# StractOrg/stract

Measured on NVIDIA H100. Metric: webgraph_edges_per_sec_per_centrality_iter, higher is better.
Workload: dtype u8

## Files before the change

### stract_b200/csrc/api_graph.cu

```cuda
#include "graph.cuh"

#include <algorithm>
#include <vector>

namespace sb200 {
static thread_local char t_err[1024] = "";
std::atomic<uint64_t> g_launches{0};
thread_local cudaStream_t t_pool_stream = nullptr;
void set_error(const char* fmt, ...) {
  va_list ap; va_start(ap, fmt);
  vsnprintf(t_err, sizeof(t_err), fmt, ap);
  va_end(ap);
}
int hb_alloc_state(sb200_graph* g);
int hb_reset(sb200_graph* g);
int hb_step(sb200_graph* g, sb200_iter_stats* st);
int hb_step_launch(sb200_graph* g, bool with_barrier);
int hb_step_finish(sb200_graph* g, sb200_iter_stats* st);
int hb_barrier(sb200_graph* g);
__global__ void k_owned_flags(const uint32_t* __restrict__ inv, const uint32_t* __restrict__ sub, uint64_t N, uint32_t world, uint32_t rank,
                              uint8_t* owned, uint32_t* sub_out) {
  const uint64_t r = blockIdx.x * (uint64_t)blockDim.x + threadIdx.x;
  if (r >= N) return;
  const uint32_t v = inv[r];
  if (owned) owned[r] = (world <= 1 || ((v >> 5) % world) == rank) ? 1 : 0;
  if (sub_out) sub_out[r] = sub ? sub[v] : (world <= 1 ? 1u : 0xFFFFFFFFu >> (32 - world));
}
int hb_result(sb200_graph* g, uint64_t* id_lo, uint64_t* id_hi, double* cent, uint64_t cap, uint64_t* len);
int hb_registers(sb200_graph* g, uint64_t first, uint64_t count, uint8_t* out);
int hb_ranked(sb200_graph* g, int ties_desc, uint64_t* id_lo, uint64_t* id_hi, double* cent, uint64_t cap, uint64_t* len);
int hb_kahan(sb200_graph* g, uint64_t first, uint64_t count, double* sum, double* err);
}
using namespace sb200;

uint64_t sb200_graph::hbm_bytes() const {
  return id_lo.bytes() + id_hi.bytes() + perm.bytes() + inv.bytes() + row_ptr.bytes() + col.bytes() + fwd_ptr.bytes() +
         fwd_dst.bytes() + item_row.bytes() + item_start.bytes() + partial.bytes() + regs[0].bytes() + regs[1].bytes() +
         bm[0].bytes() + bm[1].bytes() + size_cache.bytes() + kahan_sum.bytes() + kahan_err.bytes() +
         frontier_list.bytes() + frontier_off.bytes() + frontier_scan.bytes() + cub_tmp.bytes() + counters.bytes() + sub_mask.bytes() + sync_page.bytes();
}

extern "C" {

const char* sb200_last_error(void) { return t_err; }
#ifndef SB200_EMU
const char* sb200_version(void) { return "stract_b200 0.1 (sm_90a)"; }
#else
const char* sb200_version(void) { return "stract_b200 0.1 CPU SIMT emulation (tests/emu, tests only)"; }
#endif
uint64_t sb200_kernel_launch_count(void) { return g_launches.load(); }

#define SB_ENTER(g)                                            \
  if (!(g)) SB_FAIL(SB200_EINVAL, "NULL graph handle");        \
  SB_CUDA(cudaSetDevice((g)->device))

int sb200_graph_create(const uint64_t* from_lo, const uint64_t* from_hi, const uint64_t* to_lo, const uint64_t* to_hi,
                       const uint64_t* rel_flags, uint64_t n_edges, uint64_t skipped_rel_mask, int device, int rank,
                       int world_size, sb200_graph** out) {
  if (!out) SB_FAIL(SB200_EINVAL, "out is NULL");
  *out = nullptr;
  if (world_size < 1 || world_size > 64 || rank < 0 || rank >= world_size)
// ... 106 lines not shown
  SB_CUDA(cudaEventRecord(g->ev_run1, g->stream));
  SB_CUDA(cudaStreamSynchronize(g->stream));
  cudaEventElapsedTime(&g->last_run_ms, g->ev_run0, g->ev_run1);
  if (iters_done) *iters_done = g->t;
  return SB200_OK;
}

int sb200_hyperball_last_run_ms(sb200_graph* g, float* ms) {
  if (!g || !ms) SB_FAIL(SB200_EINVAL, "NULL argument");
  *ms = g->last_run_ms;
  return SB200_OK;
}

int sb200_hyperball_set_profiling(sb200_graph* g, int on) {
  if (!g) SB_FAIL(SB200_EINVAL, "NULL graph handle");
  g->profiling = on != 0;
  for (int f = 0; f < sb200_graph::F_COUNT; f++) { g->prof_launches[f] = 0; g->prof_ms[f] = 0; g->prof_bytes[f] = 0; g->prof_used[f] = false; }
  return SB200_OK;
}

int sb200_hyperball_get_profile(sb200_graph* g, sb200_kernel_prof* out, uint32_t cap, uint32_t* n) {
  if (!g || !n) SB_FAIL(SB200_EINVAL, "NULL argument");
  static const char* names[sb200_graph::F_COUNT] = {"k_pull_warp<dense>", "k_pull_quad<dense>", "k_pull_warp<frontier>",
                                                     "k_pull_quad<frontier>", "k_pull_merge", "k_push", "k_finalize"};
  uint32_t k = 0;
  for (int f = 0; f < sb200_graph::F_COUNT; f++) {
    if (out && k < cap) {
      memset(&out[k], 0, sizeof(out[k]));
      strncpy(out[k].name, names[f], sizeof(out[k].name) - 1);
      out[k].launches = g->prof_launches[f]; out[k].ms = g->prof_ms[f]; out[k].alg_bytes = g->prof_bytes[f];
    }
    k++;
  }
  *n = k;
  return SB200_OK;
}

int sb200_hyperball_result(sb200_graph* g, uint64_t* id_lo, uint64_t* id_hi, double* centrality, uint64_t cap, uint64_t* len) {
  SB_ENTER(g);
  if (!len) SB_FAIL(SB200_EINVAL, "len is NULL");
  if (centrality && (!id_lo || !id_hi)) SB_FAIL(SB200_EINVAL, "id outputs are NULL");
  return hb_result(g, id_lo, id_hi, centrality, cap, len);
}

int sb200_hyperball_ranked(sb200_graph* g, int ties_desc, uint64_t* id_lo, uint64_t* id_hi, double* centrality, uint64_t cap, uint64_t* len) {
  SB_ENTER(g);
  if (!len) SB_FAIL(SB200_EINVAL, "len is NULL");
// ... 229 lines not shown
```

### stract_b200/csrc/graph.cuh

```cuda
#pragma once
#include "common.cuh"

namespace sb200 {
constexpr int MAX_PEERS = 15;
struct PeerOut { uint4* newr[MAX_PEERS]; uint32_t* bmc[MAX_PEERS]; const uint32_t* sub; int n; uint32_t world, rank; uint8_t prank[MAX_PEERS + 1]; };
constexpr int SYNC_SLOTS = 128;
struct SyncView { unsigned long long* local; unsigned long long* peer[MAX_PEERS]; int n; uint32_t world, rank; };
}

struct sb200_graph {
  int device = 0, rank = 0, world = 1;
  cudaStream_t stream = nullptr;
  cudaEvent_t ev0 = nullptr, ev1 = nullptr;
  uint64_t N = 0, E_in = 0, E_kept = 0, E_local = 0;
  uint64_t row_begin = 0, row_end = 0;
  uint64_t n_pos = 0;
  bool has_fwd = false;
  int reuse = 0;
  double stage_ms = 0;

  sb200::DevBuf<uint64_t> id_lo, id_hi;
  sb200::DevBuf<uint32_t> perm, inv;
  sb200::DevBuf<uint32_t> self_bm;
  sb200::DevBuf<uint32_t> row_ptr, col;
  uint32_t col_base = 0;
  sb200::DevBuf<uint32_t> fwd_ptr, fwd_dst;
  sb200::DevBuf<uint32_t> row_ranges_host_dummy;
  uint64_t range_begins[65] = {0};

  uint64_t warp_row_begin = 0, warp_row_end = 0;
  uint64_t quad_row_begin = 0, quad_row_end = 0;
  uint64_t n_items = 0;
  uint64_t n_multi_rows = 0;
  sb200::DevBuf<uint32_t> owned_items;
  uint64_t n_owned_items = 0;
  sb200::DevBuf<uint32_t> item_row, item_start;
  sb200::DevBuf<uint4> partial;
  uint64_t n_multi_items = 0;

  sb200::DevBuf<uint8_t> regs[2];
  sb200::DevBuf<uint32_t> bm[2];
  sb200::DevBuf<uint64_t> size_cache;
  sb200::DevBuf<double> kahan_sum, kahan_err;
  sb200::DevBuf<uint32_t> frontier_list, frontier_off;
  sb200::DevBuf<unsigned long long> frontier_scan;
  sb200::DevBuf<uint8_t> cub_tmp;
  sb200::DevBuf<unsigned long long> counters;
  unsigned long long* h_counters = nullptr;
  int cur = 0;
  int bcur = 0;
  uint32_t t = 0;
  bool has_changes = true;
  uint64_t n_changed_prev = 0, frontier_edges_prev = 0;
  bool exchange_pending = false;
  int n_peers = 0;
  bool p2p = false;
  bool peers_ipc = true;
  void* peer_regs[2][sb200::MAX_PEERS] = {{nullptr}};
  void* peer_bm[2][sb200::MAX_PEERS] = {{nullptr}};
  int peer_rank[sb200::MAX_PEERS] = {0};
  bool publish_all = false;
  sb200::DevBuf<uint32_t> sub_mask;
  uint64_t n_subscribed = 0;
  sb200::DevBuf<unsigned long long> sync_page;
  void* peer_sync[sb200::MAX_PEERS] = {nullptr};
  uint64_t sync_epoch = 0;
  bool step_in_flight = false, step_with_barrier = false;
  int step_mode = 0;
  double dense_frac = 0.35, push_div = 48.0;
  int force_mode = -1;
  uint64_t l2_window_bytes = 0;

  enum { F_PULL_WARP_DENSE, F_PULL_QUAD_DENSE, F_PULL_WARP_FRONT, F_PULL_QUAD_FRONT, F_PULL_MERGE, F_PUSH, F_FINALIZE, F_COUNT };
  bool profiling = false;
  uint64_t prof_launches[F_COUNT] = {0};
  double prof_ms[F_COUNT] = {0}, prof_bytes[F_COUNT] = {0};
  cudaEvent_t prof_ev[F_COUNT][2] = {{nullptr}};
  int sm_count = 0;
  int opt_side_ctas = -1, opt_owned_list = -1;
  cudaStream_t side_stream = nullptr;
  cudaEvent_t ev_fork = nullptr, ev_join = nullptr, side_prof[2] = {nullptr, nullptr};
  bool side_prof_used = false;
  int side_prof_family = 0;
  bool prof_used[F_COUNT] = {false};
  double prof_step_bytes[F_COUNT] = {0};
  uint64_t E_warp = 0, E_quad = 0;
  double own_frac = 1.0;
  cudaEvent_t ev_run0 = nullptr, ev_run1 = nullptr;
  float last_run_ms = 0;

  uint64_t hbm_bytes() const;
};

namespace sb200 {
constexpr int QUAD_MAX_DEG = 32;
constexpr int CHUNK_EDGES = 1024;
// ... 6 lines not shown
```

### stract_b200/csrc/hyperball.cu

```cuda
#include <chrono>
#include "graph.cuh"
#include "../../include/sb200_hll_tables.h"

#ifndef SB200_EMU
#include <cub/cub.cuh>
#endif
#include <algorithm>
#include <cmath>
#include <cstdlib>

namespace sb200 {

struct HllTables {
  double raw[SB200_HLL_P5_LEN];
  double bias[SB200_HLL_P5_LEN];
  double lc[65];
};
__constant__ HllTables c_tab;
static bool g_tab_loaded[64] = {false};

int load_tables(int device) {
  if (device >= 0 && device < 64 && g_tab_loaded[device]) return SB200_OK;
  static HllTables h;
  for (int i = 0; i < SB200_HLL_P5_LEN; i++) { h.raw[i] = SB200_HLL_RAW_P5[i]; h.bias[i] = SB200_HLL_BIAS_P5[i]; }
// ... 45 lines not shown
        idx = right ? ir : il;
      } else if (il >= 0) { right = false; idx = il; }
      else { right = true; idx = ir; }
      bsum = __dadd_rn(bsum, tab->bias[idx]);
      if (right) ir = (idx < LEN - 1) ? idx + 1 : -1;
      else il = (idx > 0) ? idx - 1 : -1;
    }
    e_star = __dsub_rn(e, __ddiv_rn(bsum, 6.0));
  }
  const double h = (zeros != 0) ? tab->lc[zeros] : e_star;
  const double pick = (h <= 40.0) ? h : e_star;
  if (!(pick == pick) || pick <= 0.0) return 0ull;
  if (pick >= 18446744073709551616.0) return 0xFFFFFFFFFFFFFFFFull;
  return (uint64_t)__double2ull_rz(pick);
}

__device__ __forceinline__ void kahan_add(double& sum, double& err, double rhs) {
  const double y = __dsub_rn(rhs, err);
  const double t = __dadd_rn(sum, y);
  err = __dsub_rn(__dsub_rn(t, sum), y);
  sum = t;
}

__global__ void k_hb_init(const uint64_t* __restrict__ id_lo, const uint32_t* __restrict__ perm, uint64_t N,
                          uint4* r0, uint4* r1, uint64_t* size_cache, double* ksum, double* kerr) {
  __shared__ HllTables tab;
  for (int i = threadIdx.x; i < (int)(sizeof(HllTables) / 8); i += blockDim.x) ((double*)&tab)[i] = ((const double*)&c_tab)[i];
  __syncthreads();
  uint64_t v = blockIdx.x * (uint64_t)blockDim.x + threadIdx.x;
  if (v >= N) return;
  const uint64_t hash = id_lo[perm[v]] * 11400714819323198549ull;
  const uint32_t j = (uint32_t)(hash >> 58);
  const uint64_t wv = hash << 6;
  const uint32_t p = (wv == 0 ? 64u : (uint32_t)__clzll((long long)wv)) + 1u;
  uint32_t w[16];
#pragma unroll
  for (int i = 0; i < 16; i++) w[i] = 0;
#pragma unroll
  for (int i = 0; i < 16; i++) if ((int)(j >> 2) == i) w[i] = p << (8 * (j & 3));
#pragma unroll
  for (int q = 0; q < 4; q++) {
    uint4 x = make_uint4(w[4 * q], w[4 * q + 1], w[4 * q + 2], w[4 * q + 3]);
    r0[v * 4 + q] = x; r1[v * 4 + q] = x;
  }
  size_cache[v] = hll64_size(w, &tab);
  ksum[v] = 0.0; kerr[v] = 0.0;
}
__global__ void k_bm_fill(uint32_t* bm, uint64_t N, uint64_t words) {
  uint64_t i = blockIdx.x * (uint64_t)blockDim.x + threadIdx.x;
  if (i >= words) return;
  uint64_t first = i * 32;
  uint32_t m = 0xFFFFFFFFu;
  if (first + 32 > N) m = (N > first) ? ((1u << (N - first)) - 1u) : 0u;
  bm[i] = m;
}

__device__ __forceinline__ bool owned_row(const PeerOut& o, uint32_t row) {
  return o.world <= 1u || ((row >> 5) % o.world) == o.rank;
}
__device__ __forceinline__ void publish_row(uint4* __restrict__ newr, uint32_t* __restrict__ bm_cur, const PeerOut& peers,
                                            uint32_t row, uint32_t sub, uint4 acc, bool write, bool changed) {
  if (write) newr[(uint64_t)row * 4 + sub] = acc;
  if (changed && sub == 0) atomicOr(bm_cur + (row >> 5), 1u << (row & 31));
  if (!write || peers.n == 0) return;
  const uint32_t want = peers.sub ? __ldg(peers.sub + row) : 0xFFFFFFFFu;
  for (int p = 0; p < peers.n; p++) {
    if ((want >> peers.prank[p]) & 1u) peers.newr[p][(uint64_t)row * 4 + sub] = acc;
  }
}

__device__ __forceinline__ bool bm_test(const uint32_t* __restrict__ bm, uint32_t v) {
  return (__ldg(bm + (v >> 5)) >> (v & 31)) & 1u;
}

template <bool FRONTIER>
__device__ __forceinline__ void quad_rows(uint64_t row, bool live, uint32_t sub, uint32_t lane,
    const uint32_t* __restrict__ row_ptr, const uint32_t* __restrict__ col, uint32_t col_base,
    const uint4* __restrict__ oldr, uint4* __restrict__ newr,
    const uint32_t* __restrict__ bm_prev, uint32_t* __restrict__ bm_cur, const PeerOut& peers) {
  const uint32_t e0 = live ? row_ptr[row] - col_base : 0u, e1 = live ? row_ptr[row + 1] - col_base : 0u;
  const uint4 own = oldr[row * 4 + sub];
  uint4 acc = own;
  const unsigned qmask = 0xFu << (lane & ~3u);
  const uint32_t self = (uint32_t)row;
  uint32_t nxt = (e0 + sub < e1) ? ld_stream_u32(col + e0 + sub) : self;
  for (uint32_t e = e0; e < e1; e += 4) {
    uint32_t mine = nxt;
    nxt = (e + 4 + sub < e1) ? ld_stream_u32(col + e + 4 + sub) : self;
    if (FRONTIER) mine = bm_test(bm_prev, mine) ? mine : self;
    const uint32_t i0 = __shfl_sync(qmask, mine, 0, 4);
    const uint32_t i1 = __shfl_sync(qmask, mine, 1, 4);
    const uint32_t i2 = __shfl_sync(qmask, mine, 2, 4);
    const uint32_t i3 = __shfl_sync(qmask, mine, 3, 4);
    const uint4 v0 = oldr[(uint64_t)i0 * 4 + sub];
    const uint4 v1 = oldr[(uint64_t)i1 * 4 + sub];
    const uint4 v2 = oldr[(uint64_t)i2 * 4 + sub];
    const uint4 v3 = oldr[(uint64_t)i3 * 4 + sub];
    acc = vmax_u8x16(vmax_u8x16(acc, v0), vmax_u8x16(vmax_u8x16(v1, v2), v3));
  }
  const unsigned ball = __ballot_sync(0xffffffffu, ne_u4(acc, own));
  const bool changed = ((ball >> (lane & ~3u)) & 0xFu) != 0u;
  if (!live) return;
  publish_row(newr, bm_cur, peers, (uint32_t)row, sub, acc, changed || bm_test(bm_prev, (uint32_t)row), changed);
}

template <bool FRONTIER>
__global__ void __launch_bounds__(256, 7) k_pull_quad(uint64_t row_begin, uint64_t row_end,
    const uint32_t* __restrict__ row_ptr, const uint32_t* __restrict__ col, uint32_t col_base,
    const uint4* __restrict__ oldr, uint4* __restrict__ newr,
    const uint32_t* __restrict__ bm_prev, uint32_t* __restrict__ bm_cur, const PeerOut peers) {
  const uint64_t gt = blockIdx.x * (uint64_t)blockDim.x + threadIdx.x;
  const uint32_t sub = threadIdx.x & 3;
  const uint32_t lane = threadIdx.x & 31;
  uint64_t row = row_begin + (gt >> 2);
  bool live = row < row_end;
  if (!live) row = row_end - 1;
  live = live && owned_row(peers, (uint32_t)row);
  if (__ballot_sync(0xffffffffu, live) == 0u) return;
  quad_rows<FRONTIER>(row, live, sub, lane, row_ptr, col, col_base, oldr, newr, bm_prev, bm_cur, peers);
}

template <bool FRONTIER>
__global__ void __launch_bounds__(256, 4) k_pull_quad_owned(uint64_t row_begin, uint64_t row_end, uint64_t first_block, uint64_t n_tasks,
    const uint32_t* __restrict__ row_ptr, const uint32_t* __restrict__ col, uint32_t col_base,
    const uint4* __restrict__ oldr, uint4* __restrict__ newr,
    const uint32_t* __restrict__ bm_prev, uint32_t* __restrict__ bm_cur, const PeerOut peers) {
  const uint32_t sub = threadIdx.x & 3, lane = threadIdx.x & 31;
  const uint64_t warps = (uint64_t)gridDim.x * (blockDim.x >> 5);
  for (uint64_t task = ((uint64_t)blockIdx.x * blockDim.x + threadIdx.x) >> 5; task < n_tasks; task += warps) {
    const uint64_t block = first_block + (task >> 2) * peers.world;
    uint64_t row = block * 32 + (task & 3) * 8 + (lane >> 2);
    const bool live = row >= row_begin && row < row_end;
    if (!live) row = row_begin;
    if (__ballot_sync(0xffffffffu, live) == 0u) continue;
    quad_rows<FRONTIER>(row, live, sub, lane, row_ptr, col, col_base, oldr, newr, bm_prev, bm_cur, peers);
  }
}

template <bool FRONTIER>
__global__ void __launch_bounds__(256, 4) k_pull_quad2(uint64_t row_begin, uint64_t row_end,
    const uint32_t* __restrict__ row_ptr, const uint32_t* __restrict__ col,
    const uint4* __restrict__ oldr, uint4* __restrict__ newr,
    const uint32_t* __restrict__ bm_prev, uint32_t* __restrict__ bm_cur) {
  const uint64_t gt = blockIdx.x * (uint64_t)blockDim.x + threadIdx.x;
  const uint32_t sub = threadIdx.x & 3, lane = threadIdx.x & 31;
  const uint64_t pair = gt >> 2;
  uint64_t rowA = row_begin + 2 * pair, rowB = rowA + 1;
  const bool liveA = rowA < row_end, liveB = rowB < row_end;
  if (!liveA) rowA = row_end - 1;
  if (!liveB) rowB = row_end - 1;
  if (__ballot_sync(0xffffffffu, liveA) == 0u) return;
  const uint32_t a0 = liveA ? row_ptr[rowA] : 0u, a1 = liveA ? row_ptr[rowA + 1] : 0u;
  const uint32_t b0 = liveB ? row_ptr[rowB] : 0u, b1 = liveB ? row_ptr[rowB + 1] : 0u;
  uint4 accA = oldr[rowA * 4 + sub], accB = oldr[rowB * 4 + sub];
  const unsigned qmask = 0xFu << (lane & ~3u);
  const uint32_t selfA = (uint32_t)rowA, selfB = (uint32_t)rowB;
  const uint32_t steps = max((a1 - a0 + 3u) >> 2, (b1 - b0 + 3u) >> 2);
  uint32_t nA = (a0 + sub < a1) ? ld_stream_u32(col + a0 + sub) : selfA;
  uint32_t nB = (b0 + sub < b1) ? ld_stream_u32(col + b0 + sub) : selfB;
  for (uint32_t i = 0; i < steps; i++) {
    uint32_t mA = nA, mB = nB;
    const uint32_t ea = a0 + 4 * (i + 1) + sub, eb = b0 + 4 * (i + 1) + sub;
    nA = (ea < a1) ? ld_stream_u32(col + ea) : selfA;
    nB = (eb < b1) ? ld_stream_u32(col + eb) : selfB;
    if (FRONTIER) { mA = bm_test(bm_prev, mA) ? mA : selfA; mB = bm_test(bm_prev, mB) ? mB : selfB; }
    const uint32_t iA0 = __shfl_sync(qmask, mA, 0, 4), iA1 = __shfl_sync(qmask, mA, 1, 4), iA2 = __shfl_sync(qmask, mA, 2, 4), iA3 = __shfl_sync(qmask, mA, 3, 4);
    const uint32_t iB0 = __shfl_sync(qmask, mB, 0, 4), iB1 = __shfl_sync(qmask, mB, 1, 4), iB2 = __shfl_sync(qmask, mB, 2, 4), iB3 = __shfl_sync(qmask, mB, 3, 4);
    const uint4 vA0 = oldr[(uint64_t)iA0 * 4 + sub], vA1 = oldr[(uint64_t)iA1 * 4 + sub], vA2 = oldr[(uint64_t)iA2 * 4 + sub], vA3 = oldr[(uint64_t)iA3 * 4 + sub];
    const uint4 vB0 = oldr[(uint64_t)iB0 * 4 + sub], vB1 = oldr[(uint64_t)iB1 * 4 + sub], vB2 = oldr[(uint64_t)iB2 * 4 + sub], vB3 = oldr[(uint64_t)iB3 * 4 + sub];
    accA = vmax_u8x16(vmax_u8x16(accA, vA0), vmax_u8x16(vmax_u8x16(vA1, vA2), vA3));
    accB = vmax_u8x16(vmax_u8x16(accB, vB0), vmax_u8x16(vmax_u8x16(vB1, vB2), vB3));
  }
  const uint4 ownA = oldr[rowA * 4 + sub], ownB = oldr[rowB * 4 + sub];
  const unsigned ballA = __ballot_sync(0xffffffffu, ne_u4(accA, ownA)), ballB = __ballot_sync(0xffffffffu, ne_u4(accB, ownB));
  const bool chA = ((ballA >> (lane & ~3u)) & 0xFu) != 0u, chB = ((ballB >> (lane & ~3u)) & 0xFu) != 0u;
  if (liveA && (chA || bm_test(bm_prev, selfA))) newr[rowA * 4 + sub] = accA;
  if (liveA && chA && sub == 0) atomicOr(bm_cur + (selfA >> 5), 1u << (selfA & 31));
  if (liveB && (chB || bm_test(bm_prev, selfB))) newr[rowB * 4 + sub] = accB;
  if (liveB && chB && sub == 0) atomicOr(bm_cur + (selfB >> 5), 1u << (selfB & 31));
}

template <bool FRONTIER, bool LISTED>
__global__ void __launch_bounds__(256, 8) k_pull_warp(uint64_t n_items, uint64_t first_multi_free_item,
    const uint32_t* __restrict__ item_list, const uint32_t* __restrict__ item_row, const uint32_t* __restrict__ item_start, uint32_t warp_row_begin,
    const uint32_t* __restrict__ row_ptr, const uint32_t* __restrict__ col, uint32_t col_base,
    const uint4* __restrict__ oldr, uint4* __restrict__ newr, uint4* __restrict__ partial,
    const uint32_t* __restrict__ bm_prev, uint32_t* __restrict__ bm_cur, const PeerOut peers) {
  uint64_t item = (blockIdx.x * (uint64_t)blockDim.x + threadIdx.x) >> 5;
  if (item >= n_items) return;
  if (LISTED) item = item_list[item];
  const uint32_t lane = threadIdx.x & 31, sub = lane & 3, q = lane >> 2;
  const uint32_t row = item_row[item];
  if (!owned_row(peers, row)) return;
  const uint32_t chunk = (uint32_t)item - item_start[row - warp_row_begin];
  const uint32_t rs = row_ptr[row] - col_base, re = row_ptr[row + 1] - col_base;
  const uint32_t e0 = rs + chunk * (uint32_t)CHUNK_EDGES;
  const uint32_t e1 = min(e0 + (uint32_t)CHUNK_EDGES, re);
  uint4 acc = make_uint4(0, 0, 0, 0);
  uint32_t nxt = (e0 + lane < e1) ? ld_stream_u32(col + e0 + lane) : row;
  for (uint32_t base = e0; base < e1; base += 32) {
    uint32_t mine = nxt;
    nxt = (base + 32 + lane < e1) ? ld_stream_u32(col + base + 32 + lane) : row;
    if (FRONTIER) mine = bm_test(bm_prev, mine) ? mine : row;
    const uint32_t i0 = __shfl_sync(0xffffffffu, mine, q);
    const uint32_t i1 = __shfl_sync(0xffffffffu, mine, q + 8);
    const uint32_t i2 = __shfl_sync(0xffffffffu, mine, q + 16);
    const uint32_t i3 = __shfl_sync(0xffffffffu, mine, q + 24);
    const uint4 v0 = oldr[(uint64_t)i0 * 4 + sub];
    const uint4 v1 = oldr[(uint64_t)i1 * 4 + sub];
    const uint4 v2 = oldr[(uint64_t)i2 * 4 + sub];
    const uint4 v3 = oldr[(uint64_t)i3 * 4 + sub];
    acc = vmax_u8x16(vmax_u8x16(acc, v0), vmax_u8x16(vmax_u8x16(v1, v2), v3));
  }
#pragma unroll
  for (int off = 4; off < 32; off <<= 1) {
    uint4 o;
    o.x = __shfl_xor_sync(0xffffffffu, acc.x, off); o.y = __shfl_xor_sync(0xffffffffu, acc.y, off);
    o.z = __shfl_xor_sync(0xffffffffu, acc.z, off); o.w = __shfl_xor_sync(0xffffffffu, acc.w, off);
    acc = vmax_u8x16(acc, o);
  }
  if (item < first_multi_free_item) {
    if (q == 0) partial[item * 4 + sub] = acc;
    return;
  }
  const uint4 own = oldr[(uint64_t)row * 4 + sub];
  acc = vmax_u8x16(acc, own);
  const unsigned ball = __ballot_sync(0xffffffffu, ne_u4(acc, own));
  const bool changed = (ball & 0xFu) != 0u;
  if (q == 0) publish_row(newr, bm_cur, peers, row, sub, acc, changed || bm_test(bm_prev, row), changed);
}

__global__ void __launch_bounds__(256) k_pull_merge(uint64_t n_rows, const uint32_t* __restrict__ item_start,
    uint32_t warp_row_begin, const uint4* __restrict__ partial, const uint4* __restrict__ oldr,
    uint4* __restrict__ newr, const uint32_t* __restrict__ bm_prev, uint32_t* __restrict__ bm_cur, const PeerOut peers) {
  const uint64_t r = (blockIdx.x * (uint64_t)blockDim.x + threadIdx.x) >> 5;
  if (r >= n_rows) return;
  const uint32_t lane = threadIdx.x & 31, sub = lane & 3, q = lane >> 2;
  const uint32_t row = warp_row_begin + (uint32_t)r;
  if (!owned_row(peers, row)) return;
  const uint32_t i0 = item_start[r], i1 = item_start[r + 1];
  uint4 acc = make_uint4(0, 0, 0, 0);
  for (uint32_t it = i0 + q; it < i1; it += 8) acc = vmax_u8x16(acc, partial[(uint64_t)it * 4 + sub]);
#pragma unroll
  for (int off = 4; off < 32; off <<= 1) {
    uint4 o;
    o.x = __shfl_xor_sync(0xffffffffu, acc.x, off); o.y = __shfl_xor_sync(0xffffffffu, acc.y, off);
    o.z = __shfl_xor_sync(0xffffffffu, acc.z, off); o.w = __shfl_xor_sync(0xffffffffu, acc.w, off);
    acc = vmax_u8x16(acc, o);
// ... 224 lines not shown
}
__global__ void k_gather_f64x2(const uint32_t* __restrict__ inv, const double* __restrict__ a, const double* __restrict__ b,
                               uint64_t first, uint64_t count, double* oa, double* ob) {
  uint64_t i = blockIdx.x * (uint64_t)blockDim.x + threadIdx.x;
  if (i >= count) return;
  uint32_t v = inv[first + i];
  oa[i] = a[v]; ob[i] = b[v];
}

static double env_f(const char* name, double dflt) {
  const char* s = getenv(name);
  return s ? atof(s) : dflt;
}

int hb_alloc_state(sb200_graph* g) {
  g->dense_frac = env_f("SB200_DENSE_FRAC", g->dense_frac);
  g->push_div = env_f("SB200_PUSH_DIV", g->push_div);
  g->force_mode = (int)env_f("SB200_FORCE_MODE", (double)g->force_mode);
  const uint64_t N = g->N;
  const uint64_t words = (N + 31) / 32;
  SB_TRY(load_tables(g->device));
  SB_TRY(g->regs[0].alloc(std::max<uint64_t>(N, 1) * 64));
  SB_TRY(g->regs[1].alloc(std::max<uint64_t>(N, 1) * 64));
  SB_TRY(g->bm[0].alloc(words + 1)); SB_TRY(g->bm[1].alloc(words + 1));
  SB_TRY(g->size_cache.alloc(std::max<uint64_t>(N, 1)));
  SB_TRY(g->kahan_sum.alloc(std::max<uint64_t>(N, 1))); SB_TRY(g->kahan_err.alloc(std::max<uint64_t>(N, 1)));
  SB_TRY(g->counters.alloc(8));
  if (g->world > 1) {
    SB_TRY(g->sync_page.alloc(SYNC_SLOTS));
    SB_CUDA(cudaMemset(g->sync_page.p, 0, SYNC_SLOTS * sizeof(unsigned long long)));
    g->publish_all = env_flag("SB200_PUBLISH_ALL", false);
  }
  if (!g->h_counters) SB_CUDA(cudaMallocHost((void**)&g->h_counters, 8 * sizeof(unsigned long long)));
  const double mb = env_f("SB200_L2_PERSIST_MB", 16.0);
  g->l2_window_bytes = 0;
  if (mb > 0) {
    cudaDeviceProp prop;
    SB_CUDA(cudaGetDeviceProperties(&prop, g->device));
    uint64_t want = (uint64_t)(mb * 1048576.0);
    want = std::min<uint64_t>(want, (uint64_t)std::max(prop.persistingL2CacheMaxSize, 0));
    want = std::min<uint64_t>(want, (uint64_t)std::max(prop.accessPolicyMaxWindowSize, 0));
    want = std::min<uint64_t>(want, N * 64);
    if (want) { SB_CUDA(cudaDeviceSetLimit(cudaLimitPersistingL2CacheSize, want)); g->l2_window_bytes = want; }
  }
  return SB200_OK;
}

int hb_reset(sb200_graph* g) {
  cudaStream_t s = g->stream;
  const uint64_t N = g->N, words = (N + 31) / 32;
  g->cur = 0; g->bcur = 0; g->t = 0; g->has_changes = N > 0; g->exchange_pending = false;
  g->n_changed_prev = N; g->frontier_edges_prev = g->E_kept;
  if (N == 0) return SB200_OK;
  SB_LAUNCH(k_hb_init, div_up(N, 256), 256, 0, s, g->id_lo.p, g->perm.p, N, (uint4*)g->regs[0].p, (uint4*)g->regs[1].p,
            g->size_cache.p, g->kahan_sum.p, g->kahan_err.p);
  SB_CHECK_LAUNCH();
  SB_LAUNCH(k_bm_fill, div_up(words, 256), 256, 0, s, g->bm[0].p, N, words);
  SB_CHECK_LAUNCH();
  SB_CUDA(cudaMemsetAsync(g->bm[1].p, 0, (words + 1) * 4, s));
  SB_CUDA(cudaStreamSynchronize(s));
  return SB200_OK;
}

#define PROF_BEGIN(g, fam) do { if ((g)->profiling) { SB_CUDA(cudaEventRecord((g)->prof_ev[fam][0], (g)->stream)); } } while (0)
#define PROF_END(g, fam, bytes) do { if ((g)->profiling) { SB_CUDA(cudaEventRecord((g)->prof_ev[fam][1], (g)->stream)); \
    (g)->prof_used[fam] = true; (g)->prof_step_bytes[fam] = (double)(bytes); } } while (0)

static PeerOut make_peer_out(const sb200_graph* g, bool with_targets) {
  PeerOut po;
  memset(&po, 0, sizeof(po));
  po.world = (uint32_t)g->world; po.rank = (uint32_t)g->rank;
  if (with_targets && g->p2p) {
    po.n = g->n_peers;
    po.sub = (g->publish_all || !g->sub_mask.p) ? nullptr : g->sub_mask.p;
    for (int p = 0; p < g->n_peers; p++) {
      po.newr[p] = (uint4*)g->peer_regs[g->cur ^ 1][p]; po.bmc[p] = (uint32_t*)g->peer_bm[g->bcur ^ 1][p];
      po.prank[p] = (uint8_t)g->peer_rank[p];
    }
  }
  return po;
}

template <bool FRONTIER>
static int launch_pull(sb200_graph* g, const uint4* oldr, uint4* newr, const uint32_t* bmp, uint32_t* bmc) {
  cudaStream_t s = g->stream;
  const PeerOut po = make_peer_out(g, true);
  const int FW = FRONTIER ? sb200_graph::F_PULL_WARP_FRONT : sb200_graph::F_PULL_WARP_DENSE;
  const int FQ = FRONTIER ? sb200_graph::F_PULL_QUAD_FRONT : sb200_graph::F_PULL_QUAD_DENSE;
  const double per_edge = FRONTIER ? 4.0 : 68.0;
  if (g->opt_side_ctas < 0) {
    const bool multicast_target = g->n_peers < g->world - 1;
    g->opt_side_ctas = (int)env_f("SB200_QUAD_SIDE_CTAS", (multicast_target || g->world <= 4) ? 2.0 : 0.0);
  }
  const int side_ctas = g->opt_side_ctas;
  const bool side_quad = side_ctas > 0 && g->world > 1 && g->p2p && g->n_peers > 0 && g->n_items && g->quad_row_end > g->quad_row_begin;
  if (side_quad) {
    if (!g->side_stream) {
      int lo = 0, hi = 0;
      SB_CUDA(cudaDeviceGetStreamPriorityRange(&lo, &hi));
      SB_CUDA(cudaStreamCreateWithPriority(&g->side_stream, cudaStreamNonBlocking, hi));
      SB_CUDA(cudaEventCreateWithFlags(&g->ev_fork, cudaEventDisableTiming));
      SB_CUDA(cudaEventCreateWithFlags(&g->ev_join, cudaEventDisableTiming));
      SB_CUDA(cudaEventCreate(&g->side_prof[0])); SB_CUDA(cudaEventCreate(&g->side_prof[1]));
    }
    if (!g->sm_count) SB_CUDA(cudaDeviceGetAttribute(&g->sm_count, cudaDevAttrMultiProcessorCount, g->device));
    const int sm_count = g->sm_count;
    const uint64_t world = (uint64_t)g->world, b0 = g->quad_row_begin >> 5, b1 = (g->quad_row_end - 1) >> 5;
    const uint64_t first = b0 + ((uint64_t)g->rank + world - b0 % world) % world;
    const uint64_t n_tasks = first <= b1 ? ((b1 - first) / world + 1) * 4 : 0;
    SB_CUDA(cudaEventRecord(g->ev_fork, s));
    SB_CUDA(cudaStreamWaitEvent(g->side_stream, g->ev_fork, 0));
    if (g->l2_window_bytes) {
      cudaStreamAttrValue a;
      memset(&a, 0, sizeof(a));
      a.accessPolicyWindow.base_ptr = (void*)oldr; a.accessPolicyWindow.num_bytes = g->l2_window_bytes;
      a.accessPolicyWindow.hitRatio = 1.0f; a.accessPolicyWindow.hitProp = cudaAccessPropertyPersisting;
      a.accessPolicyWindow.missProp = cudaAccessPropertyStreaming;
      SB_CUDA(cudaStreamSetAttribute(g->side_stream, cudaStreamAttributeAccessPolicyWindow, &a));
    }
    if (g->profiling) SB_CUDA(cudaEventRecord(g->side_prof[0], g->side_stream));
    if (getenv("SB200_DEBUG_SIDE")) fprintf(stderr, "[sb200] side quad: rank %d tasks %llu\n", g->rank, (unsigned long long)n_tasks);
    if (n_tasks) {
      const unsigned grid = (unsigned)std::min<uint64_t>(div_up(n_tasks, 8), (uint64_t)sm_count * (uint64_t)side_ctas);
      SB_LAUNCH(k_pull_quad_owned<FRONTIER>, grid, 256, 0, g->side_stream, g->quad_row_begin, g->quad_row_end, first, n_tasks,
                g->row_ptr.p, g->col.p, g->col_base, oldr, newr, bmp, bmc, po);
      SB_CHECK_LAUNCH();
    }
    if (g->profiling) {
      SB_CUDA(cudaEventRecord(g->side_prof[1], g->side_stream));
      g->side_prof_used = true; g->side_prof_family = FQ;
      g->prof_step_bytes[FQ] = g->own_frac * (per_edge * (double)g->E_quad + 68.0 * (double)(g->quad_row_end - g->quad_row_begin));
    }
  }
  if (g->n_items) {
    PROF_BEGIN(g, FW);
    if (g->opt_owned_list < 0) g->opt_owned_list = env_flag("SB200_OWNED_ITEMS", true) ? 1 : 0;
    const bool listed = g->opt_owned_list > 0 && g->world > 1 && g->owned_items.p;
    const uint64_t n_launch = listed ? g->n_owned_items : g->n_items;
    auto kern = listed ? k_pull_warp<FRONTIER, true> : k_pull_warp<FRONTIER, false>;
    if (n_launch)
    SB_LAUNCH(kern, div_up(n_launch * 32, 256), 256, 0, s, n_launch, g->n_multi_items,
              listed ? g->owned_items.p : (const uint32_t*)nullptr, g->item_row.p, g->item_start.p, (uint32_t)g->warp_row_begin, g->row_ptr.p, g->col.p, g->col_base, oldr, newr,
              g->partial.p, bmp, bmc, po);
    SB_CHECK_LAUNCH();
    PROF_END(g, FW, g->own_frac * (per_edge * (double)g->E_warp + 68.0 * (double)(g->warp_row_end - g->warp_row_begin - g->n_multi_rows)));
  }
  if (g->n_multi_rows) {
    PROF_BEGIN(g, sb200_graph::F_PULL_MERGE);
    SB_LAUNCH(k_pull_merge, div_up(g->n_multi_rows * 32, 256), 256, 0, s, g->n_multi_rows, g->item_start.p,
              (uint32_t)g->warp_row_begin, g->partial.p, oldr, newr, bmp, bmc, po);
    SB_CHECK_LAUNCH();
    PROF_END(g, sb200_graph::F_PULL_MERGE, 64.0 * (double)g->n_multi_items + 68.0 * (double)g->n_multi_rows);
  }
  const uint64_t nq = g->quad_row_end - g->quad_row_begin;
  if (side_quad) { SB_CUDA(cudaEventRecord(g->ev_join, g->side_stream)); SB_CUDA(cudaStreamWaitEvent(s, g->ev_join, 0)); }
  else if (nq) {
    PROF_BEGIN(g, FQ);
    static const bool quad2 = env_flag("SB200_QUAD2", false);
    if (quad2 && g->world == 1 && g->col_base == 0)
      SB_LAUNCH(k_pull_quad2<FRONTIER>, div_up(((nq + 1) / 2) * 4, 256), 256, 0, s, g->quad_row_begin, g->quad_row_end, g->row_ptr.p,
                g->col.p, oldr, newr, bmp, bmc);
    else
    SB_LAUNCH(k_pull_quad<FRONTIER>, div_up(nq * 4, 256), 256, 0, s, g->quad_row_begin, g->quad_row_end, g->row_ptr.p,
              g->col.p, g->col_base, oldr, newr, bmp, bmc, po);
    SB_CHECK_LAUNCH();
    PROF_END(g, FQ, g->own_frac * (per_edge * (double)g->E_quad + 68.0 * (double)nq));
  }
  return SB200_OK;
}

static int run_push(sb200_graph* g, const uint4* oldr, uint4* newr, const uint32_t* bmp, uint32_t* bmc) {
  cudaStream_t s = g->stream;
  const uint64_t N = g->N, words = (N + 31) / 32;
  const uint64_t nf = g->n_changed_prev;
  if (nf == 0) return SB200_OK;
  if (g->frontier_list.n < 2 * (nf + 1)) { SB_TRY(g->frontier_list.alloc(2 * (nf + 1) + (nf >> 1))); }
  if (g->frontier_off.n < nf + 1) { SB_TRY(g->frontier_off.alloc(nf + 1 + (nf >> 2))); }
  if (g->frontier_scan.n < 2 * (words + 1)) { SB_TRY(g->frontier_scan.alloc(2 * (words + 1))); }
  uint32_t* list = g->frontier_list.p;
  uint32_t* fbeg = g->frontier_list.p + g->frontier_list.n / 2;
  unsigned long long* word_sum = g->frontier_scan.p;
  unsigned long long* word_pos = g->frontier_scan.p + (words + 1);
  SB_LAUNCH(k_frontier_count, div_up(words + 1, 256), 256, 0, s, bmp, words, g->fwd_ptr.p, word_sum);
  SB_CHECK_LAUNCH();
  size_t need = 0;
  SB_CUDA(cub::DeviceScan::ExclusiveSum(nullptr, need, word_sum, word_pos, (int64_t)(words + 1), s));
  if (g->cub_tmp.n < need) SB_TRY(g->cub_tmp.alloc(need + 256));
// ... 152 lines not shown
      SB_CUDA(cudaStreamSynchronize(s));
      g->frontier_edges_prev = fe0;
    }
    if (g->has_fwd) {
      const double fe = (double)g->frontier_edges_prev;
      if (fe >= dense_frac * E) mode = 0;
      else if (fe * push_div <= E) mode = 2;
      else mode = 1;
    } else {
      mode = ((double)g->n_changed_prev >= 0.75 * (double)N) ? 0 : 1;
    }
  } else {
    static const bool auto_push = env_flag("SB200_SHARDED_PUSH", true);
    const bool tiny = (double)g->n_changed_prev * 16.0 <= (double)N;
    if (!g->has_fwd && ((auto_push && g->reuse > 0 && g->t > 0 && tiny) || force_mode == 2)) SB_TRY(build_fwd_csr(g));
    if (g->has_fwd && tiny) mode = 2;
    else mode = ((double)g->n_changed_prev >= 0.75 * (double)N) ? 0 : 1;
  }
  if (force_mode >= 0 && (force_mode < 2 || g->has_fwd)) mode = force_mode;
  g->step_mode = mode;
  SB_CUDA(cudaEventRecord(g->ev0, s));
  if (!g->p2p) SB_CUDA(cudaMemsetAsync(bmc, 0, (words + 1) * 4, s));
  SB_CUDA(cudaMemsetAsync(g->counters.p, 0, 8 * sizeof(unsigned long long), s));
  if (g->l2_window_bytes && mode != 2) {
    cudaStreamAttrValue a;
    memset(&a, 0, sizeof(a));
    a.accessPolicyWindow.base_ptr = (void*)oldr; a.accessPolicyWindow.num_bytes = g->l2_window_bytes;
    a.accessPolicyWindow.hitRatio = 1.0f; a.accessPolicyWindow.hitProp = cudaAccessPropertyPersisting;
    a.accessPolicyWindow.missProp = cudaAccessPropertyStreaming;
    SB_CUDA(cudaStreamSetAttribute(s, cudaStreamAttributeAccessPolicyWindow, &a));
  }
  if (mode == 0) SB_TRY(launch_pull<false>(g, oldr, newr, bmp, bmc));
  else if (mode == 1) SB_TRY(launch_pull<true>(g, oldr, newr, bmp, bmc));
  else SB_TRY(run_push(g, oldr, newr, bmp, bmc));
  if (g->p2p && g->n_peers > 0) {
    const PeerOut po = make_peer_out(g, true);
    SB_LAUNCH(k_publish_bitmap, div_up(words, 256), 256, 0, s, bmc, words, po);
    SB_CHECK_LAUNCH();
  }
  const uint64_t nrows = g->row_end - g->row_begin;
  if (nrows) {
    PROF_BEGIN(g, sb200_graph::F_FINALIZE);
    if (!g->sm_count) SB_CUDA(cudaDeviceGetAttribute(&g->sm_count, cudaDevAttrMultiProcessorCount, g->device));
    const unsigned fin_grid = (unsigned)std::min<uint64_t>(div_up(div_up(nrows, (uint64_t)std::max(g->world, 1)), 256) + 1, (uint64_t)g->sm_count * 8);
    SB_LAUNCH(k_finalize, fin_grid, 256, 0, s, g->row_begin, g->row_end, newr, bmp, bmc, g->size_cache.p,
              g->kahan_sum.p, g->kahan_err.p, g->has_fwd ? g->fwd_ptr.p : (const uint32_t*)nullptr, (double)(g->t + 1),
              g->counters.p, (uint32_t)g->world, (uint32_t)g->rank);
    SB_CHECK_LAUNCH();
    PROF_END(g, sb200_graph::F_FINALIZE, 0.25 * (double)nrows);
  }
  if (g->p2p) SB_CUDA(cudaMemsetAsync((void*)bmp, 0, (words + 1) * 4, s));
  if (with_barrier) {
    if (!g->sync_page.p || g->n_peers != g->world - 1) SB_FAIL(SB200_ESTATE, "device barrier needs the sync pages of all %d peers", g->world - 1);
    g->sync_epoch++;
    SB_LAUNCH(k_barrier_count, 1, 32, 0, s, make_sync_view(g), (unsigned long long)g->sync_epoch, (const unsigned long long*)g->counters.p,
              g->counters.p + 5, 20000000000ull);
// ... 183 lines not shown
```

Before: 74.22 billion.

## Gather compact 16-bit seeds instead of 64-byte registers on first iteration

At init each node's single nonzero HLL register is stored as a 16-bit (index, value) seed. On iteration zero the pull kernels gather these 2-byte seeds per neighbour and expand them into register slices in registers, instead of loading 64-byte register rows. The L2 persistence window points at the seed array for that iteration. This cuts first-iteration gather traffic at the cost of an extra N*2-byte buffer and more kernel template variants.

```diff
diff --git a/stract_b200/csrc/api_graph.cu b/stract_b200/csrc/api_graph.cu
--- a/stract_b200/csrc/api_graph.cu
+++ b/stract_b200/csrc/api_graph.cu
@@ -36,7 +36,7 @@
 uint64_t sb200_graph::hbm_bytes() const {
   return id_lo.bytes() + id_hi.bytes() + perm.bytes() + inv.bytes() + row_ptr.bytes() + col.bytes() + fwd_ptr.bytes() +
          fwd_dst.bytes() + item_row.bytes() + item_start.bytes() + partial.bytes() + regs[0].bytes() + regs[1].bytes() +
-         bm[0].bytes() + bm[1].bytes() + size_cache.bytes() + kahan_sum.bytes() + kahan_err.bytes() +
+         seed.bytes() + bm[0].bytes() + bm[1].bytes() + size_cache.bytes() + kahan_sum.bytes() + kahan_err.bytes() +
          frontier_list.bytes() + frontier_off.bytes() + frontier_scan.bytes() + cub_tmp.bytes() + counters.bytes() + sub_mask.bytes() + sync_page.bytes();
 }
 
@@ -189,7 +189,8 @@
 int sb200_hyperball_get_profile(sb200_graph* g, sb200_kernel_prof* out, uint32_t cap, uint32_t* n) {
   if (!g || !n) SB_FAIL(SB200_EINVAL, "NULL argument");
   static const char* names[sb200_graph::F_COUNT] = {"k_pull_warp<dense>", "k_pull_quad<dense>", "k_pull_warp<frontier>",
-                                                     "k_pull_quad<frontier>", "k_pull_merge", "k_push", "k_finalize"};
+                                                     "k_pull_quad<frontier>", "k_pull_merge", "k_push", "k_finalize",
+                                                     "k_pull_warp<seed>", "k_pull_quad<seed>"};
   uint32_t k = 0;
   for (int f = 0; f < sb200_graph::F_COUNT; f++) {
     if (out && k < cap) {
diff --git a/stract_b200/csrc/graph.cuh b/stract_b200/csrc/graph.cuh
--- a/stract_b200/csrc/graph.cuh
+++ b/stract_b200/csrc/graph.cuh
@@ -39,6 +39,7 @@
   uint64_t n_multi_items = 0;
 
   sb200::DevBuf<uint8_t> regs[2];
+  sb200::DevBuf<uint16_t> seed;
   sb200::DevBuf<uint32_t> bm[2];
   sb200::DevBuf<uint64_t> size_cache;
   sb200::DevBuf<double> kahan_sum, kahan_err;
@@ -71,7 +72,8 @@
   int force_mode = -1;
   uint64_t l2_window_bytes = 0;
 
-  enum { F_PULL_WARP_DENSE, F_PULL_QUAD_DENSE, F_PULL_WARP_FRONT, F_PULL_QUAD_FRONT, F_PULL_MERGE, F_PUSH, F_FINALIZE, F_COUNT };
+  enum { F_PULL_WARP_DENSE, F_PULL_QUAD_DENSE, F_PULL_WARP_FRONT, F_PULL_QUAD_FRONT, F_PULL_MERGE, F_PUSH, F_FINALIZE,
+         F_PULL_WARP_SEED, F_PULL_QUAD_SEED, F_COUNT };
   bool profiling = false;
   uint64_t prof_launches[F_COUNT] = {0};
   double prof_ms[F_COUNT] = {0}, prof_bytes[F_COUNT] = {0};
diff --git a/stract_b200/csrc/hyperball.cu b/stract_b200/csrc/hyperball.cu
--- a/stract_b200/csrc/hyperball.cu
+++ b/stract_b200/csrc/hyperball.cu
@@ -91,8 +91,14 @@
   sum = t;
 }
 
+__device__ __forceinline__ uint4 seed_slice(uint32_t s, uint32_t sub) {
+  const uint32_t j = s & 63u;
+  const uint32_t v = ((j >> 4) == sub) ? (s >> 8) << (8 * (j & 3u)) : 0u;
+  const uint32_t w = (j >> 2) & 3u;
+  return make_uint4(w == 0u ? v : 0u, w == 1u ? v : 0u, w == 2u ? v : 0u, w == 3u ? v : 0u);
+}
 __global__ void k_hb_init(const uint64_t* __restrict__ id_lo, const uint32_t* __restrict__ perm, uint64_t N,
-                          uint4* r0, uint4* r1, uint64_t* size_cache, double* ksum, double* kerr) {
+                          uint4* r0, uint4* r1, uint16_t* seed, uint64_t* size_cache, double* ksum, double* kerr) {
   __shared__ HllTables tab;
   for (int i = threadIdx.x; i < (int)(sizeof(HllTables) / 8); i += blockDim.x) ((double*)&tab)[i] = ((const double*)&c_tab)[i];
   __syncthreads();
@@ -102,15 +108,14 @@
   const uint32_t j = (uint32_t)(hash >> 58);
   const uint64_t wv = hash << 6;
   const uint32_t p = (wv == 0 ? 64u : (uint32_t)__clzll((long long)wv)) + 1u;
+  const uint32_t s = j | p << 8;
+  seed[v] = (uint16_t)s;
   uint32_t w[16];
 #pragma unroll
-  for (int i = 0; i < 16; i++) w[i] = 0;
-#pragma unroll
-  for (int i = 0; i < 16; i++) if ((int)(j >> 2) == i) w[i] = p << (8 * (j & 3));
-#pragma unroll
   for (int q = 0; q < 4; q++) {
-    uint4 x = make_uint4(w[4 * q], w[4 * q + 1], w[4 * q + 2], w[4 * q + 3]);
+    const uint4 x = seed_slice(s, (uint32_t)q);
     r0[v * 4 + q] = x; r1[v * 4 + q] = x;
+    w[4 * q] = x.x; w[4 * q + 1] = x.y; w[4 * q + 2] = x.z; w[4 * q + 3] = x.w;
   }
   size_cache[v] = hll64_size(w, &tab);
   ksum[v] = 0.0; kerr[v] = 0.0;
@@ -142,17 +147,33 @@
   return (__ldg(bm + (v >> 5)) >> (v & 31)) & 1u;
 }
 
-template <bool FRONTIER>
+template <bool FRONTIER, bool SEED>
 __device__ __forceinline__ void quad_rows(uint64_t row, bool live, uint32_t sub, uint32_t lane,
     const uint32_t* __restrict__ row_ptr, const uint32_t* __restrict__ col, uint32_t col_base,
-    const uint4* __restrict__ oldr, uint4* __restrict__ newr,
+    const uint4* __restrict__ oldr, const uint16_t* __restrict__ seed, uint4* __restrict__ newr,
     const uint32_t* __restrict__ bm_prev, uint32_t* __restrict__ bm_cur, const PeerOut& peers) {
+  static_assert(!(FRONTIER && SEED), "the seed iteration gathers every source");
   const uint32_t e0 = live ? row_ptr[row] - col_base : 0u, e1 = live ? row_ptr[row + 1] - col_base : 0u;
-  const uint4 own = oldr[row * 4 + sub];
+  const uint4 own = SEED ? seed_slice(__ldg(seed + row), sub) : oldr[row * 4 + sub];
   uint4 acc = own;
   const unsigned qmask = 0xFu << (lane & ~3u);
   const uint32_t self = (uint32_t)row;
   uint32_t nxt = (e0 + sub < e1) ? ld_stream_u32(col + e0 + sub) : self;
+  if (SEED) {
+    uint32_t sn = __ldg(seed + nxt);
+    nxt = (e0 + 4 + sub < e1) ? ld_stream_u32(col + e0 + 4 + sub) : self;
+    for (uint32_t e = e0; e < e1; e += 4) {
+      const uint32_t mine = sn;
+      sn = __ldg(seed + nxt);
+      nxt = (e + 8 + sub < e1) ? ld_stream_u32(col + e + 8 + sub) : self;
+      const uint32_t s0 = __shfl_sync(qmask, mine, 0, 4);
+      const uint32_t s1 = __shfl_sync(qmask, mine, 1, 4);
+      const uint32_t s2 = __shfl_sync(qmask, mine, 2, 4);
+      const uint32_t s3 = __shfl_sync(qmask, mine, 3, 4);
+      acc = vmax_u8x16(vmax_u8x16(acc, seed_slice(s0, sub)),
+                       vmax_u8x16(vmax_u8x16(seed_slice(s1, sub), seed_slice(s2, sub)), seed_slice(s3, sub)));
+    }
+  } else
   for (uint32_t e = e0; e < e1; e += 4) {
     uint32_t mine = nxt;
     nxt = (e + 4 + sub < e1) ? ld_stream_u32(col + e + 4 + sub) : self;
@@ -173,10 +194,10 @@
   publish_row(newr, bm_cur, peers, (uint32_t)row, sub, acc, changed || bm_test(bm_prev, (uint32_t)row), changed);
 }
 
-template <bool FRONTIER>
+template <bool FRONTIER, bool SEED>
 __global__ void __launch_bounds__(256, 7) k_pull_quad(uint64_t row_begin, uint64_t row_end,
     const uint32_t* __restrict__ row_ptr, const uint32_t* __restrict__ col, uint32_t col_base,
-    const uint4* __restrict__ oldr, uint4* __restrict__ newr,
+    const uint4* __restrict__ oldr, const uint16_t* __restrict__ seed, uint4* __restrict__ newr,
     const uint32_t* __restrict__ bm_prev, uint32_t* __restrict__ bm_cur, const PeerOut peers) {
   const uint64_t gt = blockIdx.x * (uint64_t)blockDim.x + threadIdx.x;
   const uint32_t sub = threadIdx.x & 3;
@@ -186,13 +207,13 @@
   if (!live) row = row_end - 1;
   live = live && owned_row(peers, (uint32_t)row);
   if (__ballot_sync(0xffffffffu, live) == 0u) return;
-  quad_rows<FRONTIER>(row, live, sub, lane, row_ptr, col, col_base, oldr, newr, bm_prev, bm_cur, peers);
-}
-
-template <bool FRONTIER>
+  quad_rows<FRONTIER, SEED>(row, live, sub, lane, row_ptr, col, col_base, oldr, seed, newr, bm_prev, bm_cur, peers);
+}
+
+template <bool FRONTIER, bool SEED>
 __global__ void __launch_bounds__(256, 4) k_pull_quad_owned(uint64_t row_begin, uint64_t row_end, uint64_t first_block, uint64_t n_tasks,
     const uint32_t* __restrict__ row_ptr, const uint32_t* __restrict__ col, uint32_t col_base,
-    const uint4* __restrict__ oldr, uint4* __restrict__ newr,
+    const uint4* __restrict__ oldr, const uint16_t* __restrict__ seed, uint4* __restrict__ newr,
     const uint32_t* __restrict__ bm_prev, uint32_t* __restrict__ bm_cur, const PeerOut peers) {
   const uint32_t sub = threadIdx.x & 3, lane = threadIdx.x & 31;
   const uint64_t warps = (uint64_t)gridDim.x * (blockDim.x >> 5);
@@ -202,7 +223,7 @@
     const bool live = row >= row_begin && row < row_end;
     if (!live) row = row_begin;
     if (__ballot_sync(0xffffffffu, live) == 0u) continue;
-    quad_rows<FRONTIER>(row, live, sub, lane, row_ptr, col, col_base, oldr, newr, bm_prev, bm_cur, peers);
+    quad_rows<FRONTIER, SEED>(row, live, sub, lane, row_ptr, col, col_base, oldr, seed, newr, bm_prev, bm_cur, peers);
   }
 }
 
@@ -249,12 +270,13 @@
   if (liveB && chB && sub == 0) atomicOr(bm_cur + (selfB >> 5), 1u << (selfB & 31));
 }
 
-template <bool FRONTIER, bool LISTED>
+template <bool FRONTIER, bool LISTED, bool SEED>
 __global__ void __launch_bounds__(256, 8) k_pull_warp(uint64_t n_items, uint64_t first_multi_free_item,
     const uint32_t* __restrict__ item_list, const uint32_t* __restrict__ item_row, const uint32_t* __restrict__ item_start, uint32_t warp_row_begin,
     const uint32_t* __restrict__ row_ptr, const uint32_t* __restrict__ col, uint32_t col_base,
-    const uint4* __restrict__ oldr, uint4* __restrict__ newr, uint4* __restrict__ partial,
+    const uint4* __restrict__ oldr, const uint16_t* __restrict__ seed, uint4* __restrict__ newr, uint4* __restrict__ partial,
     const uint32_t* __restrict__ bm_prev, uint32_t* __restrict__ bm_cur, const PeerOut peers) {
+  static_assert(!(FRONTIER && SEED), "the seed iteration gathers every source");
   uint64_t item = (blockIdx.x * (uint64_t)blockDim.x + threadIdx.x) >> 5;
   if (item >= n_items) return;
   if (LISTED) item = item_list[item];
@@ -267,6 +289,21 @@
   const uint32_t e1 = min(e0 + (uint32_t)CHUNK_EDGES, re);
   uint4 acc = make_uint4(0, 0, 0, 0);
   uint32_t nxt = (e0 + lane < e1) ? ld_stream_u32(col + e0 + lane) : row;
+  if (SEED) {
+    uint32_t sn = __ldg(seed + nxt);
+    nxt = (e0 + 32 + lane < e1) ? ld_stream_u32(col + e0 + 32 + lane) : row;
+    for (uint32_t base = e0; base < e1; base += 32) {
+      const uint32_t mine = sn;
+      sn = __ldg(seed + nxt);
+      nxt = (base + 64 + lane < e1) ? ld_stream_u32(col + base + 64 + lane) : row;
+      const uint32_t s0 = __shfl_sync(0xffffffffu, mine, q);
+      const uint32_t s1 = __shfl_sync(0xffffffffu, mine, q + 8);
+      const uint32_t s2 = __shfl_sync(0xffffffffu, mine, q + 16);
+      const uint32_t s3 = __shfl_sync(0xffffffffu, mine, q + 24);
+      acc = vmax_u8x16(vmax_u8x16(acc, seed_slice(s0, sub)),
+                       vmax_u8x16(vmax_u8x16(seed_slice(s1, sub), seed_slice(s2, sub)), seed_slice(s3, sub)));
+    }
+  } else
   for (uint32_t base = e0; base < e1; base += 32) {
     uint32_t mine = nxt;
     nxt = (base + 32 + lane < e1) ? ld_stream_u32(col + base + 32 + lane) : row;
@@ -292,7 +329,7 @@
     if (q == 0) partial[item * 4 + sub] = acc;
     return;
   }
-  const uint4 own = oldr[(uint64_t)row * 4 + sub];
+  const uint4 own = SEED ? seed_slice(__ldg(seed + row), sub) : oldr[(uint64_t)row * 4 + sub];
   acc = vmax_u8x16(acc, own);
   const unsigned ball = __ballot_sync(0xffffffffu, ne_u4(acc, own));
   const bool changed = (ball & 0xFu) != 0u;
@@ -563,6 +600,7 @@
   SB_TRY(load_tables(g->device));
   SB_TRY(g->regs[0].alloc(std::max<uint64_t>(N, 1) * 64));
   SB_TRY(g->regs[1].alloc(std::max<uint64_t>(N, 1) * 64));
+  SB_TRY(g->seed.alloc(std::max<uint64_t>(N, 1)));
   SB_TRY(g->bm[0].alloc(words + 1)); SB_TRY(g->bm[1].alloc(words + 1));
   SB_TRY(g->size_cache.alloc(std::max<uint64_t>(N, 1)));
   SB_TRY(g->kahan_sum.alloc(std::max<uint64_t>(N, 1))); SB_TRY(g->kahan_err.alloc(std::max<uint64_t>(N, 1)));
@@ -594,7 +632,7 @@
   g->n_changed_prev = N; g->frontier_edges_prev = g->E_kept;
   if (N == 0) return SB200_OK;
   SB_LAUNCH(k_hb_init, div_up(N, 256), 256, 0, s, g->id_lo.p, g->perm.p, N, (uint4*)g->regs[0].p, (uint4*)g->regs[1].p,
-            g->size_cache.p, g->kahan_sum.p, g->kahan_err.p);
+            g->seed.p, g->size_cache.p, g->kahan_sum.p, g->kahan_err.p);
   SB_CHECK_LAUNCH();
   SB_LAUNCH(k_bm_fill, div_up(words, 256), 256, 0, s, g->bm[0].p, N, words);
   SB_CHECK_LAUNCH();
@@ -622,13 +660,27 @@
   return po;
 }
 
-template <bool FRONTIER>
+static int set_l2_window(cudaStream_t s, const void* base, uint64_t bytes) {
+  cudaStreamAttrValue a;
+  memset(&a, 0, sizeof(a));
+  a.accessPolicyWindow.base_ptr = (void*)base; a.accessPolicyWindow.num_bytes = bytes;
+  a.accessPolicyWindow.hitRatio = 1.0f; a.accessPolicyWindow.hitProp = cudaAccessPropertyPersisting;
+  a.accessPolicyWindow.missProp = cudaAccessPropertyStreaming;
+  SB_CUDA(cudaStreamSetAttribute(s, cudaStreamAttributeAccessPolicyWindow, &a));
+  return SB200_OK;
+}
+static void l2_window_of(const sb200_graph* g, const uint4* oldr, bool from_seed, const void** base, uint64_t* bytes) {
+  *base = from_seed ? (const void*)g->seed.p : (const void*)oldr;
+  *bytes = from_seed ? std::min<uint64_t>(g->l2_window_bytes, g->N * sizeof(uint16_t)) : g->l2_window_bytes;
+}
+
+template <bool FRONTIER, bool SEED>
 static int launch_pull(sb200_graph* g, const uint4* oldr, uint4* newr, const uint32_t* bmp, uint32_t* bmc) {
   cudaStream_t s = g->stream;
   const PeerOut po = make_peer_out(g, true);
-  const int FW = FRONTIER ? sb200_graph::F_PULL_WARP_FRONT : sb200_graph::F_PULL_WARP_DENSE;
-  const int FQ = FRONTIER ? sb200_graph::F_PULL_QUAD_FRONT : sb200_graph::F_PULL_QUAD_DENSE;
-  const double per_edge = FRONTIER ? 4.0 : 68.0;
+  const int FW = SEED ? sb200_graph::F_PULL_WARP_SEED : FRONTIER ? sb200_graph::F_PULL_WARP_FRONT : sb200_graph::F_PULL_WARP_DENSE;
+  const int FQ = SEED ? sb200_graph::F_PULL_QUAD_SEED : FRONTIER ? sb200_graph::F_PULL_QUAD_FRONT : sb200_graph::F_PULL_QUAD_DENSE;
+  const double per_edge = SEED ? 6.0 : FRONTIER ? 4.0 : 68.0;
   if (g->opt_side_ctas < 0) {
     const bool multicast_target = g->n_peers < g->world - 1;
     g->opt_side_ctas = (int)env_f("SB200_QUAD_SIDE_CTAS", (multicast_target || g->world <= 4) ? 2.0 : 0.0);
@@ -652,19 +704,17 @@
     SB_CUDA(cudaEventRecord(g->ev_fork, s));
     SB_CUDA(cudaStreamWaitEvent(g->side_stream, g->ev_fork, 0));
     if (g->l2_window_bytes) {
-      cudaStreamAttrValue a;
-      memset(&a, 0, sizeof(a));
-      a.accessPolicyWindow.base_ptr = (void*)oldr; a.accessPolicyWindow.num_bytes = g->l2_window_bytes;
-      a.accessPolicyWindow.hitRatio = 1.0f; a.accessPolicyWindow.hitProp = cudaAccessPropertyPersisting;
-      a.accessPolicyWindow.missProp = cudaAccessPropertyStreaming;
-      SB_CUDA(cudaStreamSetAttribute(g->side_stream, cudaStreamAttributeAccessPolicyWindow, &a));
+      const void* wbase; uint64_t wbytes;
+      l2_window_of(g, oldr, SEED, &wbase, &wbytes);
+      SB_TRY(set_l2_window(g->side_stream, wbase, wbytes));
     }
     if (g->profiling) SB_CUDA(cudaEventRecord(g->side_prof[0], g->side_stream));
     if (getenv("SB200_DEBUG_SIDE")) fprintf(stderr, "[sb200] side quad: rank %d tasks %llu\n", g->rank, (unsigned long long)n_tasks);
     if (n_tasks) {
       const unsigned grid = (unsigned)std::min<uint64_t>(div_up(n_tasks, 8), (uint64_t)sm_count * (uint64_t)side_ctas);
-      SB_LAUNCH(k_pull_quad_owned<FRONTIER>, grid, 256, 0, g->side_stream, g->quad_row_begin, g->quad_row_end, first, n_tasks,
-                g->row_ptr.p, g->col.p, g->col_base, oldr, newr, bmp, bmc, po);
+      auto kern = k_pull_quad_owned<FRONTIER, SEED>;
+      SB_LAUNCH(kern, grid, 256, 0, g->side_stream, g->quad_row_begin, g->quad_row_end, first, n_tasks,
+                g->row_ptr.p, g->col.p, g->col_base, oldr, g->seed.p, newr, bmp, bmc, po);
       SB_CHECK_LAUNCH();
     }
     if (g->profiling) {
@@ -678,11 +728,11 @@
     if (g->opt_owned_list < 0) g->opt_owned_list = env_flag("SB200_OWNED_ITEMS", true) ? 1 : 0;
     const bool listed = g->opt_owned_list > 0 && g->world > 1 && g->owned_items.p;
     const uint64_t n_launch = listed ? g->n_owned_items : g->n_items;
-    auto kern = listed ? k_pull_warp<FRONTIER, true> : k_pull_warp<FRONTIER, false>;
+    auto kern = listed ? k_pull_warp<FRONTIER, true, SEED> : k_pull_warp<FRONTIER, false, SEED>;
     if (n_launch)
     SB_LAUNCH(kern, div_up(n_launch * 32, 256), 256, 0, s, n_launch, g->n_multi_items,
-              listed ? g->owned_items.p : (const uint32_t*)nullptr, g->item_row.p, g->item_start.p, (uint32_t)g->warp_row_begin, g->row_ptr.p, g->col.p, g->col_base, oldr, newr,
-              g->partial.p, bmp, bmc, po);
+              listed ? g->owned_items.p : (const uint32_t*)nullptr, g->item_row.p, g->item_start.p, (uint32_t)g->warp_row_begin, g->row_ptr.p, g->col.p, g->col_base, oldr,
+              g->seed.p, newr, g->partial.p, bmp, bmc, po);
     SB_CHECK_LAUNCH();
     PROF_END(g, FW, g->own_frac * (per_edge * (double)g->E_warp + 68.0 * (double)(g->warp_row_end - g->warp_row_begin - g->n_multi_rows)));
   }
@@ -698,12 +748,13 @@
   else if (nq) {
     PROF_BEGIN(g, FQ);
     static const bool quad2 = env_flag("SB200_QUAD2", false);
-    if (quad2 && g->world == 1 && g->col_base == 0)
+    auto kern = k_pull_quad<FRONTIER, SEED>;
+    if (quad2 && !SEED && g->world == 1 && g->col_base == 0)
       SB_LAUNCH(k_pull_quad2<FRONTIER>, div_up(((nq + 1) / 2) * 4, 256), 256, 0, s, g->quad_row_begin, g->quad_row_end, g->row_ptr.p,
                 g->col.p, oldr, newr, bmp, bmc);
     else
-    SB_LAUNCH(k_pull_quad<FRONTIER>, div_up(nq * 4, 256), 256, 0, s, g->quad_row_begin, g->quad_row_end, g->row_ptr.p,
-              g->col.p, g->col_base, oldr, newr, bmp, bmc, po);
+    SB_LAUNCH(kern, div_up(nq * 4, 256), 256, 0, s, g->quad_row_begin, g->quad_row_end, g->row_ptr.p,
+              g->col.p, g->col_base, oldr, g->seed.p, newr, bmp, bmc, po);
     SB_CHECK_LAUNCH();
     PROF_END(g, FQ, g->own_frac * (per_edge * (double)g->E_quad + 68.0 * (double)nq));
   }
@@ -902,16 +953,15 @@
   SB_CUDA(cudaEventRecord(g->ev0, s));
   if (!g->p2p) SB_CUDA(cudaMemsetAsync(bmc, 0, (words + 1) * 4, s));
   SB_CUDA(cudaMemsetAsync(g->counters.p, 0, 8 * sizeof(unsigned long long), s));
+  const bool from_seed = g->t == 0 && mode != 2;
   if (g->l2_window_bytes && mode != 2) {
-    cudaStreamAttrValue a;
-    memset(&a, 0, sizeof(a));
-    a.accessPolicyWindow.base_ptr = (void*)oldr; a.accessPolicyWindow.num_bytes = g->l2_window_bytes;
-    a.accessPolicyWindow.hitRatio = 1.0f; a.accessPolicyWindow.hitProp = cudaAccessPropertyPersisting;
-    a.accessPolicyWindow.missProp = cudaAccessPropertyStreaming;
-    SB_CUDA(cudaStreamSetAttribute(s, cudaStreamAttributeAccessPolicyWindow, &a));
-  }
-  if (mode == 0) SB_TRY(launch_pull<false>(g, oldr, newr, bmp, bmc));
-  else if (mode == 1) SB_TRY(launch_pull<true>(g, oldr, newr, bmp, bmc));
+    const void* wbase; uint64_t wbytes;
+    l2_window_of(g, oldr, from_seed, &wbase, &wbytes);
+    SB_TRY(set_l2_window(s, wbase, wbytes));
+  }
+  if (from_seed) SB_TRY((launch_pull<false, true>(g, oldr, newr, bmp, bmc)));
+  else if (mode == 0) SB_TRY((launch_pull<false, false>(g, oldr, newr, bmp, bmc)));
+  else if (mode == 1) SB_TRY((launch_pull<true, false>(g, oldr, newr, bmp, bmc)));
   else SB_TRY(run_push(g, oldr, newr, bmp, bmc));
   if (g->p2p && g->n_peers > 0) {
     const PeerOut po = make_peer_out(g, true);
```

After: 76.77 billion (median of 6 runs). 3.4% higher.
